# ARTIST-Association/ARTIST

Measured on AMD Instinct MI355X. Metric: traced rays/s fwd+bwd, 1000-heliostat NURBS field, higher is better.
Workload: dtype f32; 1 GPU; metric config: 1000 heliostats x 100 rays/point x 10000 points (1e+09 rays/step), 10x10 degree-3 NURBS, 256x256 bitmap, surface-reconstruction epoch fwd+bwd; heliostats=1000, rays_per_point=100, points_per_heliostat=10000, parallelism=heliostat-sharded dp1, heliostats_per_rank=1000

## Files before the change

artist_amd/csrc/flux_kernels.hip:

```cpp
#include <hip/hip_runtime.h>
#include <stdint.h>
#include <stdlib.h>
#include <mutex>
#include <vector>

#include "launch_common.hpp"
#include "flux_moments.hpp"

namespace art {

constexpr int kFluxBlock = 256;
constexpr int kReduceBlock = kMomentsBlock;

struct CropMap {
    float sx, sy, xc, yc;
    int W, Hh;
    __device__ __forceinline__ float ix(int j) const { return (((sx * lin11(j, W) + xc) + 1.0f) / 2.0f) * (float)(W - 1); }
    __device__ __forceinline__ float iy(int i) const { return (((sy * lin11(i, Hh) + yc) + 1.0f) / 2.0f) * (float)(Hh - 1); }
};

__device__ __forceinline__ CropMap make_map(const float* __restrict__ dims, float xc, float yc, int b, int W, int Hh, float crop_w,
                                            float crop_h)
{
    CropMap m;
// ... 112 lines not shown
#pragma unroll
        for (int q = 0; q < U; ++q) {
            if (k0 + q * (int)blockDim.x >= npx) break;
            float sx, sy;
            crop_sample_gradient(v[q], sx, sy);
            gx += (double)(go[q] * sx);
            gy += (double)(go[q] * sy);
        }
    }
    gx = block_sum(gx, s_red);
    gy = block_sum(gy, s_red);
    if (threadIdx.x == 0) finish_centre_gradient(gx, gy, W, Hh, gcom + 2 * b);
}

__device__ __forceinline__ float tap(float c, int p)
{
    const float c0 = floorf(c);
    const int p0 = (int)c0;
    const float t = c - c0;
    return p == p0 ? 1.0f - t : (p == p0 + 1 ? t : 0.0f);
}

template <int K>
__device__ __forceinline__ float gather_rows(const CropMap& m, const float* __restrict__ g, int W, int x, int y, int j0,
                                             int j1, int i0, int i1)
{
    float wx[K];
#pragma unroll
    for (int q = 0; q < K; ++q) wx[q] = j0 + q <= j1 ? tap(m.ix(j0 + q), x) : 0.0f;
    float acc = 0.0f;
    for (int i = i0; i <= i1; ++i) {
        const float wy = tap(m.iy(i), y);
        if (wy == 0.0f) continue;
        const float* __restrict__ grow = g + i * W + j0;
        float row = 0.0f;
#pragma unroll
        for (int q = 0; q < K; ++q)
            if (wx[q] != 0.0f) row += grow[q] * wx[q];
        acc += row * wy;
    }
    return acc;
}

__device__ __forceinline__ void tap_range(float scale, float centre, int n, int p, int& lo_i, int& hi_i)
{
    lo_i = 0; hi_i = n - 1;
    if (scale > 1e-6f && scale < 1e6f) {
        const float b = (centre + 1.0f) * 0.5f * (float)(n - 1) - scale * 0.5f * (float)(n - 1);
        const float lo = ((float)p - 1.004f - b) / scale, hi = ((float)p + 1.004f - b) / scale;
        if (lo > -2.0e9f && lo < 2.0e9f && hi > -2.0e9f && hi < 2.0e9f) { lo_i = max(0, (int)ceilf(lo)); hi_i = min(n - 1, (int)floorf(hi)); }
    }
}

__device__ __forceinline__ float crop_bwd_pixel(const CropMap& m, const float* __restrict__ g, float S,
                                                const float* __restrict__ gcom, int b, int Hh, int W, int x, int y)
{
    int j0, j1, i0, i1;
    tap_range(m.sx, m.xc, W, x, j0, j1);
    tap_range(m.sy, m.yc, Hh, y, i0, i1);
    float acc = 0.0f;
    if (j1 - j0 < 4) acc = gather_rows<4>(m, g, W, x, y, j0, j1, i0, i1);
    else if (j1 - j0 < 8) acc = gather_rows<8>(m, g, W, x, y, j0, j1, i0, i1);
    else {
        for (int i = i0; i <= i1; ++i) {
            const float wy = tap(m.iy(i), y);
            if (wy == 0.0f) continue;
            float row = 0.0f;
            for (int j = j0; j <= j1; ++j) {
                const float wx = tap(m.ix(j), x);
                if (wx != 0.0f) row += g[i * W + j] * wx;
            }
            acc += row * wy;
        }
    }
    return acc + gcom[2 * b] * (lin11(x, W) - m.xc) / S + gcom[2 * b + 1] * (lin11(y, Hh) - m.yc) / S;
}

constexpr int kTileX = 64, kTileY = 32, kTaps = 4, kTileRows = 64, kRowUnroll = 4;
template <bool LOSS>
__global__ __launch_bounds__(256) void flux_crop_bwd_tiled_kernel(const float* __restrict__ dims, const float* __restrict__ com,
                                                                  const float* __restrict__ gcom,
                                                                  const float* __restrict__ grad_out, int Hh, int W,
                                                                  float crop_w, float crop_h, float* __restrict__ grad_flux,
                                                                  const float* __restrict__ grad_loss, int grad_loss_stride)
{
    constexpr int CS = LOSS ? 4 : 3;
    __shared__ int s_j0[kTileX], s_i0[kTileY];
    __shared__ float s_wx[kTileX][kTaps], s_wy[kTileY][kTaps];
    __shared__ float s_t[kTileRows][kTileX];
    __shared__ int s_wide, s_ilo, s_ihi;
    __shared__ float s_gy[kTileY];
    const int b = blockIdx.z;
    const int x0 = blockIdx.x * kTileX, y0 = blockIdx.y * kTileY;
    const CropMap m = make_map(dims, com[CS * b], com[CS * b + 1], b, W, Hh, crop_w, crop_h);
    const float S = com[CS * b + 2];
    const float scale = LOSS ? (grad_loss[(int64_t)b * grad_loss_stride] * 2.0f) / com[CS * b + 3] : 1.0f;
    if (threadIdx.x == 0) { s_wide = 0; s_ilo = 0x7fffffff; s_ihi = -1; }
    __syncthreads();
    if (threadIdx.x < kTileX + kTileY) {
        const bool col = threadIdx.x < kTileX;
        const int t = col ? threadIdx.x : threadIdx.x - kTileX;
        const int p = col ? x0 + t : y0 + t;
        const int n = col ? W : Hh;
        int lo_i = 0, hi_i = -1;
        if (p < n) tap_range(col ? m.sx : m.sy, col ? m.xc : m.yc, n, p, lo_i, hi_i);
        if (hi_i - lo_i >= kTaps) s_wide = 1;
        (col ? s_j0 : s_i0)[t] = lo_i;
        for (int q = 0; q < kTaps; ++q) {
            const int o = lo_i + q;
            (col ? s_wx[t] : s_wy[t])[q] = o <= hi_i ? tap(col ? m.ix(o) : m.iy(o), p) : 0.0f;
        }
        if (!col && hi_i >= lo_i) { atomicMin(&s_ilo, lo_i); atomicMax(&s_ihi, hi_i); }
        if (!col) s_gy[t] = gcom[2 * b + 1] * (lin11(p, Hh) - m.yc) / S;
    }
    __syncthreads();
    const int ilo = s_ilo, ihi = s_ihi;
    const float* __restrict__ g = grad_out + (int64_t)b * Hh * W;
    if (s_wide || ihi - ilo >= kTileRows) {
        for (int k = threadIdx.x; k < kTileX * kTileY; k += 256) {
            const int x = x0 + (k & (kTileX - 1)), y = y0 + k / kTileX;
            if (x < W && y < Hh) grad_flux[((int64_t)b * Hh + y) * W + x] = scale * crop_bwd_pixel(m, g, S, gcom, b, Hh, W, x, y);
        }
        return;
    }
    const int tx = threadIdx.x & (kTileX - 1);
    const int x = x0 + tx;
    const bool in_x = x < W;
    const int j0 = s_j0[tx];
    const float wx0 = s_wx[tx][0], wx1 = s_wx[tx][1], wx2 = s_wx[tx][2], wx3 = s_wx[tx][3];
    const int c0 = min(j0, W - 1), c1 = min(j0 + 1, W - 1), c2 = min(j0 + 2, W - 1), c3 = min(j0 + 3, W - 1);
    const int xr = in_x ? 1 : 0;
    auto horizontal_pass = [&](auto&& row_sum) {
        for (int r = threadIdx.x / kTileX; r <= ihi - ilo; r += kRowUnroll * (256 / kTileX)) {
            float v[kRowUnroll];
#pragma unroll
            for (int q = 0; q < kRowUnroll; ++q) {
                const int rr = min(r + q * (256 / kTileX), ihi - ilo);
                v[q] = row_sum(g + (int64_t)(ilo + rr) * W);
            }
#pragma unroll
            for (int q = 0; q < kRowUnroll; ++q) {
                const int rr = r + q * (256 / kTileX);
                if (rr <= ihi - ilo) s_t[rr][tx] = in_x ? v[q] : 0.0f;
            }
        }
    };
    if (W >= 4) {
        struct __attribute__((packed, aligned(4))) Taps { float t0, t1, t2, t3; };
        const int cb = in_x ? min(j0, W - 4) : 0, sh = in_x ? j0 - cb : 0;
        const float w0 = sh == 0 ? wx0 : 0.0f, w1 = sh == 0 ? wx1 : (sh == 1 ? wx0 : 0.0f);
        const float w2 = sh == 0 ? wx2 : (sh == 1 ? wx1 : (sh == 2 ? wx0 : 0.0f));
        const float w3 = sh == 0 ? wx3 : (sh == 1 ? wx2 : (sh == 2 ? wx1 : wx0));
        horizontal_pass([&](const float* __restrict__ row) {
            const Taps t = *reinterpret_cast<const Taps*>(row + cb);
            return ((t.t0 * w0 + t.t1 * w1) + t.t2 * w2) + t.t3 * w3;
        });
    } else {
        horizontal_pass([&](const float* __restrict__ row) {
            return ((row[c0 * xr] * wx0 + row[c1 * xr] * wx1) + row[c2 * xr] * wx2) + row[c3 * xr] * wx3;
        });
    }
    __syncthreads();
    if (!in_x) return;
    const float gx = gcom[2 * b] * (lin11(x, W) - m.xc) / S;
    for (int ty = threadIdx.x / kTileX; ty < kTileY; ty += 256 / kTileX) {
        const int y = y0 + ty;
        if (y >= Hh) break;
        const int r0 = s_i0[ty] - ilo;
        float acc = 0.0f;
#pragma unroll
        for (int a = 0; a < kTaps; ++a) {
            const float wy = s_wy[ty][a];
            if (wy != 0.0f) acc += s_t[r0 + a][tx] * wy;
        }
        acc += gx + s_gy[ty];
        grad_flux[((int64_t)b * Hh + y) * W + x] = LOSS ? scale * acc : acc;
    }
}

template <typename F>
__device__ __forceinline__ void for_each_pair(const float* __restrict__ p, const float* __restrict__ g, int64_t npix, F&& f)
{
    const bool vec = (npix & 3) == 0 && ((reinterpret_cast<uintptr_t>(p) | reinterpret_cast<uintptr_t>(g)) & 15) == 0;
    if (vec) {
        const float4* __restrict__ p4 = reinterpret_cast<const float4*>(p);
        const float4* __restrict__ g4 = reinterpret_cast<const float4*>(g);
        for (int64_t k = threadIdx.x; k < (npix >> 2); k += blockDim.x) {
            const float4 a = p4[k], c = g4[k];
            f(4 * k, a.x, c.x); f(4 * k + 1, a.y, c.y); f(4 * k + 2, a.z, c.z); f(4 * k + 3, a.w, c.w);
        }
    } else {
        for (int64_t k = threadIdx.x; k < npix; k += blockDim.x) f(k, p[k], g[k]);
    }
}

struct KlNorms {
    static constexpr float eps = 1e-12f;
    float npf, ngf, dp, dg;
    __device__ __forceinline__ KlNorms(float np_, float ng_) : npf(np_), ngf(ng_), dp(fmaxf(np_, eps)), dg(fmaxf(ng_, eps)) {}
    __device__ __forceinline__ void term(float pk, float gk, double& acc, double& dot) const
    {
        const float t = logf(gk / dg + eps), q = logf(pk / dp + eps);
        const float et = expf(t);
        acc += (double)(et * (t - q));
        dot += (double)((-et / (pk / dp + eps)) * pk);
    }
    __device__ __forceinline__ float gradient(float pk, float gk, float dotf, float gl) const
    {
        const float t = logf(gk / dg + eps);
        const float a = -expf(t) / (pk / dp + eps);
        const float sgn = pk > 0.0f ? 1.0f : (pk < 0.0f ? -1.0f : 0.0f);
        const float through_norm = npf > eps ? sgn * dotf / (dp * dp) : 0.0f;
        return gl * (a / dp - through_norm);
    }
};

__global__ __launch_bounds__(kReduceBlock) void flux_loss_kernel(const float* __restrict__ pred, const float* __restrict__ truth,
                                                               int64_t npix, int mode, float* __restrict__ loss,
                                                               const float* __restrict__ grad_loss,
                                                               float* __restrict__ grad_pred)
{
    __shared__ double s_red[16];
    const int b = blockIdx.x;
    const float* __restrict__ p = pred + (int64_t)b * npix;
    const float* __restrict__ g = truth + (int64_t)b * npix;
    float* __restrict__ gp = grad_pred ? grad_pred + (int64_t)b * npix : nullptr;
    if (mode == 0) {
        double se = 0.0, sg = 0.0;
        for_each_pair(p, g, npix, [&](int64_t, float pk, float gk) { const float d = pk - gk; se += (double)(d * d); sg += (double)gk; });
        se = block_sum(se, s_red);
        const float sgf = (float)block_sum(sg, s_red);
        if (threadIdx.x == 0 && loss) loss[b] = (float)se / sgf;
        if (gp) {
            const float gl = grad_loss[b];
            for_each_pair(p, g, npix, [&](int64_t k, float pk, float gk) { gp[k] = gl * (2.0f * (pk - gk)) / sgf; });
        }
        return;
    }
    double np_ = 0.0, ng = 0.0;
    for_each_pair(p, g, npix, [&](int64_t, float pk, float gk) { np_ += (double)fabsf(pk); ng += (double)fabsf(gk); });
    const float npf = (float)block_sum(np_, s_red), ngf = (float)block_sum(ng, s_red);
    const KlNorms kl(npf, ngf);
    double acc = 0.0, dot = 0.0;
    for_each_pair(p, g, npix, [&](int64_t, float pk, float gk) { kl.term(pk, gk, acc, dot); });
    acc = block_sum(acc, s_red);
    const float dotf = (float)block_sum(dot, s_red);
    if (threadIdx.x == 0 && loss) loss[b] = (float)acc;
    if (gp) {
        const float gl = grad_loss[b];
        for_each_pair(p, g, npix, [&](int64_t k, float pk, float gk) { gp[k] = kl.gradient(pk, gk, dotf, gl); });
    }
}

constexpr int kMaxPartBitmaps = 512;
struct PartScratch { double com[kMaxPartBitmaps][kLossParts][3]; double acc[kMaxPartBitmaps][kLossParts][4]; };

__global__ __launch_bounds__(kReduceBlock) void flux_com_parts_kernel(const float* __restrict__ flux, int Hh, int W, int parts_per_wg,
                                                                    PartScratch* __restrict__ ws)
{
    __shared__ double s_red[16 * 4];
    const int b = blockIdx.y;
    const float* __restrict__ f = flux + (int64_t)b * Hh * W;
    for (int v = blockIdx.x * parts_per_wg; v < (int)(blockIdx.x + 1) * parts_per_wg; ++v) {
        double a[3];
        com_part_sums(f, Hh, W, v, s_red, a);
        if (threadIdx.x == 0) { ws->com[b][v][0] = a[0]; ws->com[b][v][1] = a[1]; ws->com[b][v][2] = a[2]; }
    }
}

__device__ __forceinline__ void com_from_parts(const double (*parts)[3], float& xc, float& yc, float& S)
{
    double s = 0.0, xs = 0.0, ys = 0.0;
    for (int v = 0; v < kLossParts; ++v) { s += parts[v][0]; xs += parts[v][1]; ys += parts[v][2]; }
    centre_from_sums(s, xs, ys, xc, yc, S);
}

__device__ __forceinline__ void loss_from_parts(const double (*acc)[4], float xc, float yc, float S, int b, int Hh, int W,
                                                float* __restrict__ loss, float* __restrict__ com4, float* __restrict__ gunit)
{
    double se = 0.0, sg = 0.0, gx = 0.0, gy = 0.0;
    for (int v = 0; v < kLossParts; ++v) { se += acc[v][0]; sg += acc[v][1]; gx += acc[v][2]; gy += acc[v][3]; }
    const float sgf = (float)sg;
    loss[b] = (float)se / sgf;
    com4[4 * b] = xc; com4[4 * b + 1] = yc; com4[4 * b + 2] = S; com4[4 * b + 3] = sgf;
    if (gunit) finish_centre_gradient(gx, gy, W, Hh, gunit + 2 * b);
}

template <bool WHOLE>
__global__ __launch_bounds__(kReduceBlock) void flux_crop_pixel_loss_fwd_kernel(const float* __restrict__ flux,
                                                                               const float* __restrict__ dims,
                                                                               const float* __restrict__ truth, int Hh, int W,
                                                                               float crop_w, float crop_h, int parts_per_wg,
                                                                               PartScratch* ws, float* __restrict__ residual,
                                                                               float* __restrict__ loss, float* __restrict__ com4,
                                                                               float* __restrict__ gunit, const double* __restrict__ moments,
                                                                               int stage_rows)
{
    extern __shared__ __attribute__((aligned(16))) float s_stage[];
    __shared__ double s_red[16 * 4];
    __shared__ double s_com[kLossParts][3], s_acc[kLossParts][4];
    const int b = blockIdx.y;
    const float* __restrict__ f = flux + (int64_t)b * Hh * W;
    const float* __restrict__ g = truth + (int64_t)b * Hh * W;
    float* __restrict__ res = residual ? residual + (int64_t)b * Hh * W : nullptr;
    float xc, yc, S;
    if (moments != nullptr) {
        com_from_parts(reinterpret_cast<const double(*)[3]>(moments + (int64_t)b * kLossParts * 3), xc, yc, S);
    } else if constexpr (WHOLE) {
        for (int v = 0; v < kLossParts; ++v) {
            double a[3];
            com_part_sums(f, Hh, W, v, s_red, a);
            if (threadIdx.x == 0) { s_com[v][0] = a[0]; s_com[v][1] = a[1]; s_com[v][2] = a[2]; }
        }
        __syncthreads();
        com_from_parts(s_com, xc, yc, S);
    } else {
        com_from_parts(ws->com[b], xc, yc, S);
    }
    const CropMap m = make_map(dims, xc, yc, b, W, Hh, crop_w, crop_h);
    for (int v = blockIdx.x * parts_per_wg; v < (int)(blockIdx.x + 1) * parts_per_wg; ++v) {
        int r0, r1;
        part_rows(Hh, v, r0, r1);
        double a[4] = {0.0, 0.0, 0.0, 0.0};
        if ((int)blockDim.x % W == 0) {
            const int j = threadIdx.x % W, di = blockDim.x / W;
            const CropAxis col = crop_column(m, j);
            int ylo = 0, nrows = 0;
            if (stage_rows > 0 && (W & 3) == 0) {
                const float ya_ = m.iy(r0), yb_ = m.iy(r1 - 1);
                if (ya_ > -1.0e9f && ya_ < 1.0e9f && yb_ > -1.0e9f && yb_ < 1.0e9f) {
                    ylo = max(0, (int)floorf(fminf(ya_, yb_)));
                    const int yhi = min(Hh - 1, (int)floorf(fmaxf(ya_, yb_)) + 1);
                    nrows = yhi - ylo + 1;
                    if (nrows > stage_rows) nrows = 0;
                }
            }
            constexpr int kRows = 4;
            auto rows = [&](auto&& pixel) {
            for (int i0 = r0 + threadIdx.x / W; i0 < r1; i0 += kRows * di) {
                float c[kRows], t[kRows], gxs[kRows], gys[kRows];
#pragma unroll
                for (int u = 0; u < kRows; ++u) {
                    const int i = min(i0 + u * di, r1 - 1);
                    CropTaps v;
                    c[u] = crop_sample_from(pixel, m, col, i, v);
                    t[u] = g[i * W + j];
                    crop_sample_gradient(v, gxs[u], gys[u]);
                }
#pragma unroll
                for (int u = 0; u < kRows; ++u) {
                    const int i = i0 + u * di;
                    if (i >= r1) break;
                    const float d = c[u] - t[u];
                    a[0] += (double)(d * d); a[1] += (double)t[u];
                    if (res) {
                        res[i * W + j] = d;
                        a[2] += (double)(d * gxs[u]);
                        a[3] += (double)(d * gys[u]);
                    }
                }
            }
            };
            if (nrows > 0) {
                __syncthreads();
                const float4* __restrict__ src = reinterpret_cast<const float4*>(f + (int64_t)ylo * W);
                float4* dst = reinterpret_cast<float4*>(s_stage);
                for (int k = threadIdx.x; k < nrows * (W >> 2); k += blockDim.x) dst[k] = src[k];
                __syncthreads();
                const float* staged = s_stage - ylo * W;
                rows([&](int k) { return staged[k]; });
            } else {
                rows([&](int k) { return f[k]; });
            }
        } else {
            for (int k = r0 * W + threadIdx.x; k < r1 * W; k += blockDim.x) {
                const int i = k / W, j = k - i * W;
                CropTaps v;
                const float c = crop_sample(f, m, crop_column(m, j), i, v);
                const float t = g[k];
                const float d = c - t;
                a[0] += (double)(d * d); a[1] += (double)t;
                if (res) {
                    float gxs, gys;
                    crop_sample_gradient(v, gxs, gys);
                    res[k] = d;
                    a[2] += (double)(d * gxs);
                    a[3] += (double)(d * gys);
                }
            }
        }
        block_sum_n<4>(a, s_red);
        if (threadIdx.x == 0) {
            double* out = WHOLE ? s_acc[v] : ws->acc[b][v];
            out[0] = a[0]; out[1] = a[1]; out[2] = a[2]; out[3] = a[3];
        }
    }
    if constexpr (WHOLE) {
        if (threadIdx.x == 0) loss_from_parts(s_acc, xc, yc, S, b, Hh, W, loss, com4, gunit);
    }
}

__global__ __launch_bounds__(256) void flux_crop_pixel_loss_final_kernel(const PartScratch* __restrict__ ws, int B, int Hh, int W,
                                                                         float* __restrict__ loss, float* __restrict__ com4,
                                                                         float* __restrict__ gunit, const double* __restrict__ moments)
{
    const int b = blockIdx.x * blockDim.x + threadIdx.x;
    if (b >= B) return;
    float xc, yc, S;
    com_from_parts(moments ? reinterpret_cast<const double(*)[3]>(moments + (int64_t)b * kLossParts * 3) : ws->com[b], xc, yc, S);
    loss_from_parts(ws->acc[b], xc, yc, S, b, Hh, W, loss, com4, gunit);
}

__global__ __launch_bounds__(kFluxBlock) void flux_com_px_bwd_kernel(const float* __restrict__ com, const float* __restrict__ grad_com,
                                                                     int Hh, int W, float* __restrict__ grad_flux)
{
    const int b = blockIdx.y;
    const int k = blockIdx.x * blockDim.x + threadIdx.x;
    if (k >= Hh * W) return;
    const int i = k / W, j = k - i * W;
    const float S = com[3 * b + 2];
    grad_flux[(int64_t)b * Hh * W + k] = (grad_com[2 * b] * ((float)j - com[3 * b]) + grad_com[2 * b + 1] * ((float)i - com[3 * b + 1])) / S;
}

template <typename F>
__device__ __forceinline__ void for_each_crop_pixel(const float* __restrict__ f, const CropMap& m, F&& fn)
{
    const int W = m.W, Hh = m.Hh;
    auto pixel = [&](int k, int i, const CropAxis& col) {
        CropTaps v;
        const float c = crop_sample(f, m, col, i, v);
        fn(k, c, v);
    };
    if ((int)blockDim.x % W == 0) {
        const int j = threadIdx.x % W, di = blockDim.x / W;
        const CropAxis col = crop_column(m, j);
#pragma unroll 4
        for (int i = threadIdx.x / W; i < Hh; i += di) pixel(i * W + j, i, col);
    } else {
        for (int k = threadIdx.x; k < Hh * W; k += blockDim.x) {
            const int i = k / W, j = k - i * W;
            pixel(k, i, crop_column(m, j));
        }
    }
}

__global__ __launch_bounds__(kReduceBlock) void flux_crop_kl_loss_fwd_kernel(const float* __restrict__ flux,
                                                                            const float* __restrict__ dims,
                                                                            const float* __restrict__ truth, int Hh, int W,
                                                                            float crop_w, float crop_h, float* __restrict__ loss,
                                                                            float* __restrict__ rec8)
{
    __shared__ double s_red[16 * 3];
    __shared__ float s_com[3];
    const int b = blockIdx.x;
    const float* __restrict__ f = flux + (int64_t)b * Hh * W;
    const float* __restrict__ g = truth + (int64_t)b * Hh * W;
    double sums[3];
// ... 11 lines not shown
    acc = block_sum(acc, s_red);
    const float dotf = (float)block_sum(dot, s_red);
    if (threadIdx.x == 0) {
        loss[b] = (float)acc;
        float* r = rec8 + 8 * b;
        r[0] = xc; r[1] = yc; r[2] = S; r[3] = npf; r[4] = ngf; r[5] = dotf; r[6] = 0.0f; r[7] = 0.0f;
    }
}

__global__ __launch_bounds__(kReduceBlock) void flux_crop_kl_loss_bwd_kernel(const float* __restrict__ flux,
                                                                            const float* __restrict__ dims,
                                                                            const float* __restrict__ truth,
                                                                            const float* __restrict__ rec8,
                                                                            const float* __restrict__ grad_loss, int Hh, int W,
                                                                            float crop_w, float crop_h,
                                                                            float* __restrict__ grad_crop, float* __restrict__ com3,
                                                                            float* __restrict__ gcom)
{
    __shared__ double s_red[16];
    const int b = blockIdx.x;
    const float* __restrict__ f = flux + (int64_t)b * Hh * W;
    const float* __restrict__ g = truth + (int64_t)b * Hh * W;
    float* __restrict__ gc = grad_crop + (int64_t)b * Hh * W;
    const float* r = rec8 + 8 * b;
    const CropMap m = make_map(dims, r[0], r[1], b, W, Hh, crop_w, crop_h);
    const KlNorms kl(r[3], r[4]);
    const float dotf = r[5], gl = grad_loss[b];
    double gx = 0.0, gy = 0.0;
    for_each_crop_pixel(f, m, [&](int k, float c, const CropTaps& v) {
        const float go = kl.gradient(c, g[k], dotf, gl);
        float sx, sy;
        crop_sample_gradient(v, sx, sy);
        gc[k] = go;
        gx += (double)(go * sx);
        gy += (double)(go * sy);
    });
    gx = block_sum(gx, s_red);
    gy = block_sum(gy, s_red);
    if (threadIdx.x == 0) {
        finish_centre_gradient(gx, gy, W, Hh, gcom + 2 * b);
        com3[3 * b] = m.xc; com3[3 * b + 1] = m.yc; com3[3 * b + 2] = r[2];
    }
}

}

using namespace art;

static PartScratch* flux_parts_scratch(hipStream_t stream)
{
    struct Entry { int dev; hipStream_t stream; PartScratch* ws; };
    static std::vector<Entry> table;
    static std::mutex lock;
    int dev = 0;
    if (hipGetDevice(&dev) != hipSuccess) return nullptr;
    std::lock_guard<std::mutex> guard(lock);
    for (const Entry& e : table)
        if (e.dev == dev && e.stream == stream) return e.ws;
    PartScratch* ws = nullptr;
    if (hipMalloc(reinterpret_cast<void**>(&ws), sizeof(PartScratch)) != hipSuccess) return nullptr;
    table.push_back({dev, stream, ws});
    return ws;
}

static int loss_workgroups_per_bitmap(int64_t B, int64_t Hh)
{
    const int forced = debug_env_int("ARTIST_HIP_LOSS_PARTS", 0);
    if (B > kMaxPartBitmaps || Hh < kLossParts) return 1;
    if (forced == 1 || forced == 2 || forced == 4) return forced;
    int cus = 256;
    {
        int dev = 0, n = 0;
        if (hipGetDevice(&dev) == hipSuccess && hipDeviceGetAttribute(&n, hipDeviceAttributeMultiprocessorCount, dev) == hipSuccess && n > 0)
            cus = n;
    }
    return 4 * B <= cus ? 4 : (2 * B <= cus ? 2 : 1);
}

template <bool LOSS>
static void launch_crop_bwd_tiled(hipStream_t stream, const float* dims, const float* com, const float* gcom, const float* grad_out,
                                  int64_t B, int64_t Hh, int64_t W, double crop_width, double crop_height, float* grad_flux,
                                  const float* grad_loss = nullptr, int64_t grad_loss_stride = 1)
{
    hipLaunchKernelGGL(flux_crop_bwd_tiled_kernel<LOSS>,
                       dim3((unsigned)((W + kTileX - 1) / kTileX), (unsigned)((Hh + kTileY - 1) / kTileY), (unsigned)B),
                       dim3(256), 0, stream, dims, com, gcom, grad_out, (int)Hh, (int)W, (float)crop_width, (float)crop_height,
                       grad_flux, grad_loss, (int)grad_loss_stride);
}

static bool crop_args_ok(const void* a, const void* b, const void* c, const void* d, int64_t B, int64_t Hh, int64_t W)
{
    return a && b && c && d && B >= 0 && Hh >= 1 && W >= 1 && Hh <= 65535 && Hh * W <= (int64_t)1 << 30 && B <= 65535;
}

static bool empty_batch(int64_t B, int64_t Hh, int64_t W)
{
    return B == 0 && Hh >= 1 && W >= 1;
}

extern "C" int art_flux_crop_fwd(const float* flux, const float* target_dims, int64_t B, int64_t Hh, int64_t W,
                                 double crop_width, double crop_height, float* out, float* centers, void* stream_)
{
    hipStream_t stream = static_cast<hipStream_t>(stream_);
    if (empty_batch(B, Hh, W)) return ART_OK;
    if (!crop_args_ok(flux, target_dims, out, centers, B, Hh, W)) return ART_EINVAL;
    hipLaunchKernelGGL(flux_com_kernel<NormalisedWeights>, dim3((unsigned)B), dim3(kReduceBlock), 0, stream, flux, (int)Hh, (int)W, centers);
    hipLaunchKernelGGL(flux_crop_fwd_kernel,
                       dim3((unsigned)((W + kFluxBlock - 1) / kFluxBlock), (unsigned)((Hh + kCropRows - 1) / kCropRows), (unsigned)B),
                       dim3(kFluxBlock), 0, stream, flux, target_dims, centers, (int)Hh, (int)W, (float)crop_width,
                       (float)crop_height, out);
    ART_HIP(hipGetLastError());
    return ART_OK;
}

extern "C" int art_flux_crop_bwd(const float* flux, const float* target_dims, const float* centers, int64_t B,
                                 int64_t Hh, int64_t W, double crop_width, double crop_height, const float* grad_out,
                                 float* grad_flux, float* workspace, void* stream_)
{
    hipStream_t stream = static_cast<hipStream_t>(stream_);
    if (empty_batch(B, Hh, W)) return ART_OK;
    if (!crop_args_ok(flux, target_dims, centers, grad_out, B, Hh, W) || !grad_flux || !workspace) return ART_EINVAL;
    hipLaunchKernelGGL(flux_crop_bwd_com_kernel, dim3((unsigned)B), dim3(kReduceBlock), 0, stream, flux, target_dims, centers,
                       grad_out, (int)Hh, (int)W, (float)crop_width, (float)crop_height, workspace);
    launch_crop_bwd_tiled<false>(stream, target_dims, centers, workspace, grad_out, B, Hh, W, crop_width, crop_height, grad_flux);
    ART_HIP(hipGetLastError());
    return ART_OK;
}

extern "C" int art_flux_loss(const float* prediction, const float* ground_truth, int64_t B, int64_t npix, int kind,
                             float* loss, const float* grad_loss, float* grad_prediction, void* stream_)
{
    hipStream_t stream = static_cast<hipStream_t>(stream_);
    if (empty_batch(B, npix, 1) && (kind == 0 || kind == 1)) return ART_OK;
    if (!prediction || !ground_truth || B < 0 || npix < 1 || (kind != 0 && kind != 1) || (!loss && !grad_prediction) ||
        (grad_prediction && !grad_loss))
        return ART_EINVAL;
    hipLaunchKernelGGL(flux_loss_kernel, dim3((unsigned)B), dim3(kReduceBlock), 0, stream, prediction, ground_truth, npix,
                       kind, loss, grad_loss, grad_prediction);
    ART_HIP(hipGetLastError());
    return ART_OK;
}

extern "C" int art_flux_crop_pixel_loss_fwd(const float* flux, const float* target_dims, const float* ground_truth, int64_t B,
                                            int64_t Hh, int64_t W, double crop_width, double crop_height, float* loss,
                                            float* centers4, float* residual, float* center_grad_unit, const double* moments,
                                            void* stream_)
{
    hipStream_t stream = static_cast<hipStream_t>(stream_);
    if (empty_batch(B, Hh, W)) return ART_OK;
    if (!crop_args_ok(flux, target_dims, ground_truth, loss, B, Hh, W) || !centers4 || (residual != nullptr) != (center_grad_unit != nullptr))
        return ART_EINVAL;
    const int P = loss_workgroups_per_bitmap(B, Hh);
    PartScratch* ws = P > 1 ? flux_parts_scratch(stream) : nullptr;
    int stage_rows = (int)std::min<int64_t>(Hh, (Hh + kLossParts - 1) / kLossParts + 4);
    if ((W & 3) != 0 || kReduceBlock % W != 0 || (int64_t)stage_rows * W * 4 > 76 * 1024) stage_rows = 0;
    const size_t stage_bytes = (size_t)stage_rows * W * sizeof(float);
    if (ws != nullptr) {
        if (moments == nullptr)
            hipLaunchKernelGGL(flux_com_parts_kernel, dim3((unsigned)P, (unsigned)B), dim3(kReduceBlock), 0, stream, flux, (int)Hh, (int)W,
                               kLossParts / P, ws);
        hipLaunchKernelGGL(flux_crop_pixel_loss_fwd_kernel<false>, dim3((unsigned)P, (unsigned)B), dim3(kReduceBlock), 0, stream, flux,
                           target_dims, ground_truth, (int)Hh, (int)W, (float)crop_width, (float)crop_height, kLossParts / P, ws, residual,
                           loss, centers4, center_grad_unit, moments, 0);
        hipLaunchKernelGGL(flux_crop_pixel_loss_final_kernel, dim3((unsigned)((B + 255) / 256)), dim3(256), 0, stream, ws, (int)B, (int)Hh,
                           (int)W, loss, centers4, center_grad_unit, moments);
    } else
    {
        if (stage_bytes > 48 * 1024)
            ART_HIP(hipFuncSetAttribute(reinterpret_cast<const void*>(&flux_crop_pixel_loss_fwd_kernel<true>),
                                        hipFuncAttributeMaxDynamicSharedMemorySize, (int)stage_bytes));
        hipLaunchKernelGGL(flux_crop_pixel_loss_fwd_kernel<true>, dim3(1u, (unsigned)B), dim3(kReduceBlock), stage_bytes, stream, flux, target_dims,
                           ground_truth, (int)Hh, (int)W, (float)crop_width, (float)crop_height, kLossParts, (PartScratch*)nullptr, residual,
                           loss, centers4, center_grad_unit, moments, stage_rows);
    }
    ART_HIP(hipGetLastError());
    return ART_OK;
}

extern "C" int art_flux_crop_pixel_loss_bwd(const float* target_dims, const float* centers4, const float* grad_loss,
                                            int64_t grad_loss_stride, const float* residual, const float* center_grad_unit, int64_t B,
                                            int64_t Hh, int64_t W, double crop_width, double crop_height, float* grad_flux, void* stream_)
{
    hipStream_t stream = static_cast<hipStream_t>(stream_);
    if (empty_batch(B, Hh, W)) return ART_OK;
    if (!crop_args_ok(residual, target_dims, center_grad_unit, centers4, B, Hh, W) || !grad_loss || !grad_flux ||
        (grad_loss_stride != 0 && grad_loss_stride != 1))
        return ART_EINVAL;
    launch_crop_bwd_tiled<true>(stream, target_dims, centers4, center_grad_unit, residual, B, Hh, W, crop_width, crop_height, grad_flux,
                                grad_loss, grad_loss_stride);
    ART_HIP(hipGetLastError());
    return ART_OK;
}

extern "C" int art_flux_center_of_mass(const float* flux, int64_t B, int64_t Hh, int64_t W, float* com, void* stream_)
{
    hipStream_t stream = static_cast<hipStream_t>(stream_);
    if (empty_batch(B, Hh, W)) return ART_OK;
    if (!crop_args_ok(flux, com, flux, com, B, Hh, W)) return ART_EINVAL;
    hipLaunchKernelGGL(flux_com_kernel<PixelWeights>, dim3((unsigned)B), dim3(kReduceBlock), 0, stream, flux, (int)Hh, (int)W, com);
    ART_HIP(hipGetLastError());
    return ART_OK;
}

extern "C" int art_flux_center_of_mass_bwd(const float* com, const float* grad_com, int64_t B, int64_t Hh, int64_t W,
                                           float* grad_flux, void* stream_)
{
    hipStream_t stream = static_cast<hipStream_t>(stream_);
    if (empty_batch(B, Hh, W)) return ART_OK;
    if (!crop_args_ok(com, grad_com, grad_flux, com, B, Hh, W)) return ART_EINVAL;
    hipLaunchKernelGGL(flux_com_px_bwd_kernel, dim3((unsigned)((Hh * W + kFluxBlock - 1) / kFluxBlock), (unsigned)B), dim3(kFluxBlock),
                       0, stream, com, grad_com, (int)Hh, (int)W, grad_flux);
    ART_HIP(hipGetLastError());
    return ART_OK;
}

extern "C" int art_flux_crop_kl_loss_fwd(const float* flux, const float* target_dims, const float* ground_truth, int64_t B,
                                         int64_t Hh, int64_t W, double crop_width, double crop_height, float* loss,
                                         float* record8, void* stream_)
{
    hipStream_t stream = static_cast<hipStream_t>(stream_);
    if (empty_batch(B, Hh, W)) return ART_OK;
    if (!crop_args_ok(flux, target_dims, ground_truth, loss, B, Hh, W) || !record8) return ART_EINVAL;
    hipLaunchKernelGGL(flux_crop_kl_loss_fwd_kernel, dim3((unsigned)B), dim3(kReduceBlock), 0, stream, flux, target_dims,
                       ground_truth, (int)Hh, (int)W, (float)crop_width, (float)crop_height, loss, record8);
    ART_HIP(hipGetLastError());
    return ART_OK;
}

extern "C" int art_flux_crop_kl_loss_bwd(const float* flux, const float* target_dims, const float* ground_truth,
                                         const float* record8, const float* grad_loss, int64_t B, int64_t Hh, int64_t W,
                                         double crop_width, double crop_height, float* grad_flux, float* workspace,
                                         void* stream_)
{
    hipStream_t stream = static_cast<hipStream_t>(stream_);
    if (empty_batch(B, Hh, W)) return ART_OK;
    if (!crop_args_ok(flux, target_dims, ground_truth, record8, B, Hh, W) || !grad_loss || !grad_flux || !workspace) return ART_EINVAL;
    float* grad_crop = workspace;
    float* com3 = workspace + B * Hh * W;
    float* gcom = com3 + 3 * B;
    hipLaunchKernelGGL(flux_crop_kl_loss_bwd_kernel, dim3((unsigned)B), dim3(kReduceBlock), 0, stream, flux, target_dims,
                       ground_truth, record8, grad_loss, (int)Hh, (int)W, (float)crop_width, (float)crop_height, grad_crop, com3,
                       gcom);
    launch_crop_bwd_tiled<false>(stream, target_dims, com3, gcom, grad_crop, B, Hh, W, crop_width, crop_height, grad_flux);
    ART_HIP(hipGetLastError());
    return ART_OK;
}
```

artist_amd/csrc/trace_kernels.hip:

```cpp
#include <hip/hip_runtime.h>
#include <algorithm>
#include <atomic>
#include <functional>
#include <cstdio>
#include <mutex>
#include <vector>
#include <stdint.h>
#include <stdlib.h>

#include <type_traits>

#define ART_TIMELINE_RECORDS_HERE
#include "trace_common.hpp"
#include "flux_moments.hpp"

namespace art {

__device__ __forceinline__ unsigned cvt_nearest_u32(float x)
{
    int q;
    asm("v_cvt_rpi_i32_f32_e32 %0, %1" : "=v"(q) : "v"(x));
    return (unsigned)q;
}

// ... 2362 lines not shown
                                                            int64_t npix, float sign_unit)
{
    const int64_t i = ((int64_t)blockIdx.x * blockDim.x + threadIdx.x) * 2;
    if (i + 1 < npix) {
        const ulonglong2 v = *reinterpret_cast<const ulonglong2*>(accum + i);
        *reinterpret_cast<float2*>(flux + i) = make_float2((float)v.x * sign_unit, (float)v.y * sign_unit);
        if ((v.x | v.y) != 0ull) *reinterpret_cast<ulonglong2*>(accum + i) = make_ulonglong2(0ull, 0ull);
    } else if (i < npix) {
        const unsigned long long v = accum[i];
        flux[i] = (float)v * sign_unit;
        if (v != 0ull) accum[i] = 0ull;
    }
}

__global__ __launch_bounds__(kMomentsBlock) void accum_to_flux_moments_kernel(unsigned long long* __restrict__ accum, float* __restrict__ flux,
                                                                             int Hh, int W, float sign_unit, double* __restrict__ moments)
{
    __shared__ double s_red[16 * 3];
    const int v = blockIdx.x;
    const int64_t map = blockIdx.y;
    unsigned long long* __restrict__ acc = accum + map * Hh * W;
    float* __restrict__ out = flux + map * Hh * W;
    auto load4 = [&](int64_t k) {
        const ulonglong2 lo = *reinterpret_cast<const ulonglong2*>(acc + 4 * k), hi = *reinterpret_cast<const ulonglong2*>(acc + 4 * k + 2);
        const float4 q = make_float4((float)lo.x * sign_unit, (float)lo.y * sign_unit, (float)hi.x * sign_unit, (float)hi.y * sign_unit);
        reinterpret_cast<float4*>(out)[k] = q;
        if ((lo.x | lo.y) != 0ull) *reinterpret_cast<ulonglong2*>(acc + 4 * k) = make_ulonglong2(0ull, 0ull);
        if ((hi.x | hi.y) != 0ull) *reinterpret_cast<ulonglong2*>(acc + 4 * k + 2) = make_ulonglong2(0ull, 0ull);
        return q;
    };
    auto load1 = [&](int64_t k) {
        const unsigned long long a1 = acc[k];
        const float q = (float)a1 * sign_unit;
        out[k] = q;
        if (a1 != 0ull) acc[k] = 0ull;
        return q;
    };
    double s, xs, ys;
    com_part_sums_from(load4, load1, Hh, W, v, s_red, s, xs, ys);
    if (threadIdx.x == 0) {
        double* m = moments + (map * kLossParts + v) * 3;
        m[0] = s; m[1] = xs; m[2] = ys;
    }
}

template <int VEC>
__global__ __launch_bounds__(256) void per_target_sum_kernel(const float* __restrict__ bitmaps,
                                                             const int32_t* __restrict__ target_idx, int H, int T,
                                                             int64_t npix, float* __restrict__ out)
{
    const int64_t i = ((int64_t)blockIdx.x * blockDim.x + threadIdx.x) * VEC;
    if (i >= npix) return;
    const int t = blockIdx.y;
    float acc[VEC];
#pragma unroll
    for (int v = 0; v < VEC; ++v) acc[v] = 0.0f;
    constexpr int kInFlight = VEC == 1 ? 64 : 8;
    for (int h0 = 0; h0 < H; h0 += kInFlight) {
        float val[kInFlight][VEC];
#pragma unroll
        for (int q = 0; q < kInFlight; ++q) {
            const int h = h0 + q;
            const bool mine = h < H && target_idx[h] == t;
#pragma unroll
            for (int v = 0; v < VEC; ++v) val[q][v] = 0.0f;
            if (mine) {
                if constexpr (VEC == 4) {
                    const float4 x = *reinterpret_cast<const float4*>(bitmaps + (int64_t)h * npix + i);
                    val[q][0] = x.x; val[q][1] = x.y; val[q][2] = x.z; val[q][3] = x.w;
                } else {
                    val[q][0] = bitmaps[(int64_t)h * npix + i];
                }
            }
        }
#pragma unroll
        for (int q = 0; q < kInFlight; ++q)
#pragma unroll
            for (int v = 0; v < VEC; ++v) acc[v] += val[q][v];
    }
#pragma unroll
    for (int v = 0; v < VEC; ++v) out[(int64_t)t * npix + i + v] = acc[v];
}

static void choose_chunks(TraceArgs& a, int target_blocks, int min_chunk)
{
    const int64_t base = (int64_t)a.H * a.n_ptiles;
    int64_t want = (target_blocks + base - 1) / (base > 0 ? base : 1);
    if (want < 1) want = 1;
    int chunk = (int)((a.R + want - 1) / want);
    if (chunk < min_chunk) chunk = min_chunk;
    if (chunk > a.R) chunk = a.R;
    a.r_chunk = chunk;
    a.n_rchunks = (a.R + chunk - 1) / chunk;
}

struct FwdConfig {
    int variant;
    int block;
    int tile_cap;
    int target_blocks;
    int min_chunk;
    int p_block;
    int p_block_bwd;
    bool p_block_fixed, p_block_bwd_fixed;
    int multipass_ratio;
    int min_rays;
    bool exact_pblock;
    int facet_points;
};

static FwdConfig fwd_config()
{
    FwdConfig c;
    const char* v = debug_env_str("ARTIST_HIP_FWD");
    c.variant = (v && v[0] == 'g') ? 1 : 0;
    c.block = debug_env_int("ARTIST_HIP_FWD_BLOCK", 1024);
    if (c.block < 64 || c.block > 1024 || (c.block % 64) != 0) c.block = 1024;
    int kb = debug_env_int("ARTIST_HIP_FWD_TILE_KB", 158);
    if (kb < 4) kb = 4;
    if (kb > 158) kb = 158;
    c.tile_cap = kb * 256;
    c.target_blocks = debug_env_int("ARTIST_HIP_FWD_BLOCKS", 512);
    c.min_chunk = debug_env_int("ARTIST_HIP_FWD_MINCHUNK", 4);
    c.min_rays = debug_env_int("ARTIST_HIP_FWD_MINRAYS", 100000);
    c.multipass_ratio = debug_env_int("ARTIST_HIP_FWD_MULTIPASS", 8);
    if (c.multipass_ratio < 1) c.multipass_ratio = 1;
    c.p_block_fixed = debug_env_str("ARTIST_HIP_FWD_PBLOCK") != nullptr;
    c.p_block_bwd_fixed = debug_env_str("ARTIST_HIP_BWD_PBLOCK") != nullptr;
    c.p_block = debug_env_int("ARTIST_HIP_FWD_PBLOCK", 1024);
    if (c.p_block < 64) c.p_block = 64;
    c.exact_pblock = debug_env_int("ARTIST_HIP_PBLOCK_EXACT", 1) != 0;
    c.facet_points = 0;
    c.p_block_bwd = debug_env_int("ARTIST_HIP_BWD_PBLOCK", 2048);
    if (c.p_block_bwd < 64) c.p_block_bwd = 64;
    return c;
}

static void window_geometry_for(TraceArgs& a, const FwdConfig& cfg, int p_block_target);

static unsigned* stream_work_counters(hipStream_t stream)
{
    struct Entry { int dev; hipStream_t stream; unsigned* base; };
    static std::vector<Entry> table;
    static unsigned* page = nullptr;
    static int page_dev = -1, page_used = 0;
    static std::mutex lock;
    constexpr int kPageEntries = 4096 / (int)(sizeof(unsigned) * kCountersPerStream);
    int dev = 0;
    if (hipGetDevice(&dev) != hipSuccess) return nullptr;
    std::lock_guard<std::mutex> guard(lock);
    for (const Entry& e : table)
        if (e.dev == dev && e.stream == stream) return e.base;
    if (page == nullptr || page_dev != dev || page_used == kPageEntries) {
        unsigned* fresh = nullptr;
        if (hipMalloc(reinterpret_cast<void**>(&fresh), 4096) != hipSuccess) return nullptr;
        if (hipMemset(fresh, 0, 4096) != hipSuccess) { (void)hipFree(fresh); return nullptr; }
        page = fresh; page_dev = dev; page_used = 0;
    }
    unsigned* base = page + (page_used++) * kCountersPerStream;
    table.push_back({dev, stream, base});
    return base;
}


struct SideStream {
    hipStream_t side = nullptr; hipEvent_t fork = nullptr, join = nullptr; int dev = -1; bool pending = false;
// ... 575 lines not shown
            const int threads = std::min(cfg.block, CY ? kCylBwdThreads : (BL ? (LN ? kLeanBlockBwdThreads : kBlockingBwdThreads) : 1024)); \
            const int rc = launch_bwd_lds<IL, AT, CY, BL, LN>(a, grad_flux, go, gn, prim_slabs, work_counter, blocks, threads, lds, stream); \
            if (rc != ART_OK) return rc;                                                                         \
        } while (0)
#define ART_LAUNCH_BWD_BL(CY, BL, LN)                                                                            \
        do {                                                                                                     \
            if (il && atomic_out) ART_LAUNCH_BWD(true, true, CY, BL, LN);                                        \
            else if (il) ART_LAUNCH_BWD(true, false, CY, BL, LN);                                                \
            else if (atomic_out) ART_LAUNCH_BWD(false, true, CY, BL, LN);                                        \
            else ART_LAUNCH_BWD(false, false, CY, BL, LN);                                                       \
        } while (0)
#define ART_LAUNCH_BWD_TYPE(CY)                                                                                  \
        do {                                                                                                     \
            if (blocking) ART_LAUNCH_BWD_BL(CY, true, false); else ART_LAUNCH_BWD_BL(CY, false, false);          \
        } while (0)
        if (T > 0 && Tc == 0 && lean) ART_LAUNCH_BWD_BL(false, false, true);
        else if (lean_block) ART_LAUNCH_BWD_BL(false, true, true);
        else
        if (T > 0 && !planar_done) ART_LAUNCH_BWD_TYPE(false);
        if (planar_done) a.split = 3;
        if (Tc > 0 && !blocking && debug_env_int("ARTIST_HIP_LEAN", 1) != 0 && debug_env_int("ARTIST_HIP_CYL_LEAN", 1) != 0) ART_LAUNCH_BWD_BL(true, false, true);
        else
        if (Tc > 0) ART_LAUNCH_BWD_TYPE(true);
#undef ART_LAUNCH_BWD_TYPE
#undef ART_LAUNCH_BWD_BL
#undef ART_LAUNCH_BWD
        ART_HIP(hipGetLastError());
        ART_HIP(diag::dump_timeline("ART_TIMELINE_OUT_BWD", items, stream));
        if (launch_lean) { const int rc = launch_lean(); if (rc != ART_OK) return rc; }
        if (blocking) {
            if (side.s) { side.s->end(); side.s = nullptr; }
            hipLaunchKernelGGL(reduce_prim_grads_kernel, dim3((unsigned)N), dim3(256), 0, stream, prim_slabs, a.wide_grad, a.cand, a.cand_count, a.H,
                               a.Cmax, a.n_pblocks * a.n_rchunks, grad_prim_corners, grad_prim_spans, grad_prim_normals);
            ART_HIP(hipGetLastError());
        }
        if (atomic_out) {
            const int64_t n = H * P;
            hipLaunchKernelGGL(reduce_chunks_kernel, dim3((unsigned)((n + 255) / 256)), dim3(256), 0, stream, go, gn, a.n_rchunks, n,
                               reinterpret_cast<float4*>(grad_origins), reinterpret_cast<float4*>(grad_normals));
            ART_HIP(hipGetLastError());
        }
        return ART_OK;
    }
    if (Tc > 0 || blocking) return ART_EUNSUPPORTED;
    a.r_chunk = a.R; a.n_rchunks = 1;
    const int64_t blocks = (int64_t)a.H * a.n_ptiles;
    if (blocks > 2147483647LL) return ART_EINVAL;
    if (il) hipLaunchKernelGGL(trace_bwd_kernel<true>, dim3((unsigned)blocks), dim3(kBlock), 0, stream, a, grad_flux, go, gn);
    else hipLaunchKernelGGL(trace_bwd_kernel<false>, dim3((unsigned)blocks), dim3(kBlock), 0, stream, a, grad_flux, go, gn);
    ART_HIP(hipGetLastError());
    return ART_OK;
}

extern "C" int64_t art_trace_bwd_scratch_need(int64_t H, int64_t R, int64_t P, int64_t facet_points, int64_t T, int64_t Tc, int64_t Cmax)
{
    if (H <= 0 || R <= 0 || P <= 0 || H > (1 << 24) || R > (1 << 24) || P > (1 << 26) || Cmax < 0 || Cmax > (1 << 22) || T < 0 || Tc < 0) return 0;
    FwdConfig cfg = fwd_config();
    if (cfg.variant != 0) return 0;
    if (facet_points < 0 || (facet_points > 0 && P % facet_points != 0)) return 0;
    const bool blocking = Cmax > 0;
    TraceArgs a = {};
    a.H = (int)H; a.R = (int)R; a.P = (int)P; a.Cmax = (int)Cmax;
    if (blocking && cfg.tile_cap > 148 * 256) cfg.tile_cap = 148 * 256;
    (void)bwd_main_geometry(a, cfg, bwd_uses_lean(blocking, T, Tc), bwd_uses_lean_block(blocking, T, Tc), facet_points, false);
    const BwdScratch n = bwd_scratch_need(a, blocking, Cmax);
    return n.chunk_floats + n.slab_floats + n.wide_floats;
}

extern "C" int64_t art_trace_bwd_scratch_floats(int64_t H, int64_t R, int64_t P, int64_t facet_points, int64_t Cmax)
{
    int64_t most = 0;
    for (int cfgno = 0; cfgno < 3; ++cfgno)
        most = std::max(most, art_trace_bwd_scratch_need(H, R, P, facet_points, cfgno == 1 ? 0 : 1, cfgno == 0 ? 0 : 1, Cmax));
    return most;
}

extern "C" int art_per_target_sum(const float* bitmaps, const int32_t* target_idx, int64_t H, int64_t T,
                                  int64_t npix, float* out, void* stream_)
{
    hipStream_t stream = static_cast<hipStream_t>(stream_);
    if (!out || T <= 0 || npix <= 0 || H < 0 || T > 65535 || (H > 0 && (!bitmaps || !target_idx))) return ART_EINVAL;
    const bool vec4 = npix >= (int64_t)1 << 20 && (npix % 4) == 0 && (reinterpret_cast<uintptr_t>(bitmaps) % 16) == 0 &&
                      (reinterpret_cast<uintptr_t>(out) % 16) == 0;
    if (vec4)
        hipLaunchKernelGGL(per_target_sum_kernel<4>, dim3((unsigned)((npix / 4 + 255) / 256), (unsigned)T), dim3(256), 0,
                           stream, bitmaps, target_idx, (int)H, (int)T, npix, out);
    else
        hipLaunchKernelGGL(per_target_sum_kernel<1>, dim3((unsigned)((npix + 255) / 256), (unsigned)T), dim3(256), 0, stream,
                           bitmaps, target_idx, (int)H, (int)T, npix, out);
    ART_HIP(hipGetLastError());
    return ART_OK;
}

extern "C" int art_async_status(void* stream_, int clear)
{
    hipStream_t stream = static_cast<hipStream_t>(stream_);
    const StatusWord status = status_word();
    if (status.host == nullptr) { g_last_hip_error = (int)hipErrorOutOfMemory; return ART_ELAUNCH; }
    ART_HIP(hipStreamSynchronize(stream));
    const unsigned word = *status.host;
    if (clear) *status.host = 0u;
    return (word & 1u) ? ART_ETARGET : ((word & 2u) ? ART_ECANDIDATES : ((word & 4u) ? ART_EQUEUE : ART_OK));
}
```

Baseline: 131.4 billion rays/s.

## Vectorize flux loss/backward stores and add strip-based per-target bitmap sum

Adds a float4-wide store path to the tiled flux crop backward kernel, and a wave-local LDS exchange in the pixel-loss forward kernel so ground-truth loads and residual stores are 16-byte coalesced. It also adds a new per-target sum kernel that has 1024-thread blocks cooperatively load many heliostat bitmaps for a 256-pixel strip, with software prefetch of the next round. The aim is to cut global memory transaction count and raise bandwidth use in these reduction and elementwise stages. The new paths raise LDS use, reduce the shared memory left for staging in the forward kernel, and are gated by alignment and env-var checks.

```diff
diff --git a/artist_amd/csrc/flux_kernels.hip b/artist_amd/csrc/flux_kernels.hip
--- a/artist_amd/csrc/flux_kernels.hip
+++ b/artist_amd/csrc/flux_kernels.hip
@@ -218,12 +218,13 @@
                                                                   const float* __restrict__ gcom,
                                                                   const float* __restrict__ grad_out, int Hh, int W,
                                                                   float crop_w, float crop_h, float* __restrict__ grad_flux,
-                                                                  const float* __restrict__ grad_loss, int grad_loss_stride)
+                                                                  const float* __restrict__ grad_loss, int grad_loss_stride,
+                                                                  int wide_store)
 {
     constexpr int CS = LOSS ? 4 : 3;
     __shared__ int s_j0[kTileX], s_i0[kTileY];
     __shared__ float s_wx[kTileX][kTaps], s_wy[kTileY][kTaps];
-    __shared__ float s_t[kTileRows][kTileX];
+    __shared__ __attribute__((aligned(16))) float s_t[kTileRows][kTileX];
     __shared__ int s_wide, s_ilo, s_ihi;
     __shared__ float s_gy[kTileY];
     const int b = blockIdx.z;
@@ -297,6 +298,36 @@
         });
     }
     __syncthreads();
+    if (wide_store) {
+        const int c4 = (threadIdx.x & 15) * 4;
+        if (x0 + c4 >= W) return;
+        float gx4[4];
+#pragma unroll
+        for (int k = 0; k < 4; ++k) gx4[k] = gcom[2 * b] * (lin11(x0 + c4 + k, W) - m.xc) / S;
+#pragma unroll
+        for (int ty = threadIdx.x >> 4; ty < kTileY; ty += 16) {
+            const int y = y0 + ty;
+            if (y >= Hh) break;
+            const int r0 = s_i0[ty] - ilo;
+            float acc[4] = {0.0f, 0.0f, 0.0f, 0.0f};
+#pragma unroll
+            for (int a = 0; a < kTaps; ++a) {
+                const float wy = s_wy[ty][a];
+                if (wy != 0.0f) {
+                    const float4 t = *reinterpret_cast<const float4*>(&s_t[r0 + a][c4]);
+                    acc[0] += t.x * wy; acc[1] += t.y * wy; acc[2] += t.z * wy; acc[3] += t.w * wy;
+                }
+            }
+            const float gy = s_gy[ty];
+#pragma unroll
+            for (int k = 0; k < 4; ++k) {
+                acc[k] += gx4[k] + gy;
+                if (LOSS) acc[k] = scale * acc[k];
+            }
+            *reinterpret_cast<float4*>(grad_flux + ((int64_t)b * Hh + y) * W + x0 + c4) = make_float4(acc[0], acc[1], acc[2], acc[3]);
+        }
+        return;
+    }
     if (!in_x) return;
     const float gx = gcom[2 * b] * (lin11(x, W) - m.xc) / S;
     for (int ty = threadIdx.x / kTileX; ty < kTileY; ty += 256 / kTileX) {
@@ -422,7 +453,7 @@
     if (gunit) finish_centre_gradient(gx, gy, W, Hh, gunit + 2 * b);
 }
 
-template <bool WHOLE>
+template <bool WHOLE, bool WIDE>
 __global__ __launch_bounds__(kReduceBlock) void flux_crop_pixel_loss_fwd_kernel(const float* __restrict__ flux,
                                                                                const float* __restrict__ dims,
                                                                                const float* __restrict__ truth, int Hh, int W,
@@ -432,6 +463,7 @@
                                                                                float* __restrict__ gunit, const double* __restrict__ moments,
                                                                                int stage_rows)
 {
+    constexpr int xchg_floats = WIDE ? kReduceBlock * 4 : 0;
     extern __shared__ __attribute__((aligned(16))) float s_stage[];
     __shared__ double s_red[16 * 4];
     __shared__ double s_com[kLossParts][3], s_acc[kLossParts][4];
@@ -458,7 +490,7 @@
         int r0, r1;
         part_rows(Hh, v, r0, r1);
         double a[4] = {0.0, 0.0, 0.0, 0.0};
-        if ((int)blockDim.x % W == 0) {
+        if (WIDE || (int)blockDim.x % W == 0) {
             const int j = threadIdx.x % W, di = blockDim.x / W;
             const CropAxis col = crop_column(m, j);
             int ylo = 0, nrows = 0;
@@ -497,18 +529,57 @@
                 }
             }
             };
+            auto rows_wide = [&](auto&& pixel) {
+                const int lane = threadIdx.x & 63, u4 = lane >> 4;
+                float* xb = s_stage + (threadIdx.x >> 6) * (kRows * 64);
+                const int c4 = (int)(threadIdx.x & ~63u) % W + 4 * (lane & 15);
+                auto segment = [&](int i0) { return min(i0 + u4 * di, r1 - 1) * W + c4; };
+                auto wave_sync = [] {
+                    __builtin_amdgcn_fence(__ATOMIC_RELEASE, "wavefront");
+                    __builtin_amdgcn_wave_barrier();
+                    __builtin_amdgcn_fence(__ATOMIC_ACQUIRE, "wavefront");
+                };
+                for (int i0 = r0 + threadIdx.x / W; i0 < r1; i0 += kRows * di) {
+                    *reinterpret_cast<float4*>(xb + 4 * lane) = *reinterpret_cast<const float4*>(g + segment(i0));
+                    wave_sync();
+                    float t[kRows];
+#pragma unroll
+                    for (int u = 0; u < kRows; ++u) t[u] = xb[u * 64 + lane];
+                    wave_sync();
+#pragma unroll
+                    for (int u = 0; u < kRows; ++u) {
+                        const int i = i0 + u * di;
+                        if (i >= r1) break;
+                        CropTaps v;
+                        float gxs, gys;
+                        const float c = crop_sample_from(pixel, m, col, i, v);
+                        crop_sample_gradient(v, gxs, gys);
+                        const float d = c - t[u];
+                        a[0] += (double)(d * d); a[1] += (double)t[u];
+                        xb[u * 64 + lane] = d;
+                        a[2] += (double)(d * gxs);
+                        a[3] += (double)(d * gys);
+                    }
+                    wave_sync();
+                    const float4 dv = *reinterpret_cast<const float4*>(xb + 4 * lane);
+                    if (i0 + u4 * di < r1) *reinterpret_cast<float4*>(res + (i0 + u4 * di) * W + c4) = dv;
+                    wave_sync();
+                }
+            };
             if (nrows > 0) {
                 __syncthreads();
                 const float4* __restrict__ src = reinterpret_cast<const float4*>(f + (int64_t)ylo * W);
-                float4* dst = reinterpret_cast<float4*>(s_stage);
+                float4* dst = reinterpret_cast<float4*>(s_stage + xchg_floats);
                 for (int k = threadIdx.x; k < nrows * (W >> 2); k += blockDim.x) dst[k] = src[k];
                 __syncthreads();
-                const float* staged = s_stage - ylo * W;
-                rows([&](int k) { return staged[k]; });
+                const float* staged = s_stage + xchg_floats - ylo * W;
+                if constexpr (WIDE) rows_wide([&](int k) { return staged[k]; });
+                else rows([&](int k) { return staged[k]; });
             } else {
-                rows([&](int k) { return f[k]; });
+                if constexpr (WIDE) rows_wide([&](int k) { return f[k]; });
+                else rows([&](int k) { return f[k]; });
             }
-        } else {
+        } else if constexpr (!WIDE) {
             for (int k = r0 * W + threadIdx.x; k < r1 * W; k += blockDim.x) {
                 const int i = k / W, j = k - i * W;
                 CropTaps v;
@@ -686,10 +757,11 @@
                                   int64_t B, int64_t Hh, int64_t W, double crop_width, double crop_height, float* grad_flux,
                                   const float* grad_loss = nullptr, int64_t grad_loss_stride = 1)
 {
+    const int wide_store = (W & 3) == 0 && (reinterpret_cast<uintptr_t>(grad_flux) & 15) == 0 && debug_env_int("ARTIST_HIP_FLUX_WIDE_BWD", 1) != 0;
     hipLaunchKernelGGL(flux_crop_bwd_tiled_kernel<LOSS>,
                        dim3((unsigned)((W + kTileX - 1) / kTileX), (unsigned)((Hh + kTileY - 1) / kTileY), (unsigned)B),
                        dim3(256), 0, stream, dims, com, gcom, grad_out, (int)Hh, (int)W, (float)crop_width, (float)crop_height,
-                       grad_flux, grad_loss, (int)grad_loss_stride);
+                       grad_flux, grad_loss, (int)grad_loss_stride, wide_store);
 }
 
 static bool crop_args_ok(const void* a, const void* b, const void* c, const void* d, int64_t B, int64_t Hh, int64_t W)
@@ -758,22 +830,27 @@
     PartScratch* ws = P > 1 ? flux_parts_scratch(stream) : nullptr;
     int stage_rows = (int)std::min<int64_t>(Hh, (Hh + kLossParts - 1) / kLossParts + 4);
     if ((W & 3) != 0 || kReduceBlock % W != 0 || (int64_t)stage_rows * W * 4 > 76 * 1024) stage_rows = 0;
-    const size_t stage_bytes = (size_t)stage_rows * W * sizeof(float);
+    const bool wide = ws == nullptr && residual != nullptr && W % 64 == 0 && kReduceBlock % W == 0 &&
+                      ((reinterpret_cast<uintptr_t>(ground_truth) | reinterpret_cast<uintptr_t>(residual)) & 15) == 0 &&
+                      debug_env_int("ARTIST_HIP_FLUX_WIDE_FWD", 1) != 0;
+    const int xchg_floats = wide ? kReduceBlock * 4 : 0;
+    if (wide && stage_rows > 0) stage_rows = (int)std::min<int64_t>(stage_rows, (76 * 1024 - xchg_floats * 4) / (W * 4));
+    const size_t stage_bytes = ((size_t)stage_rows * W + xchg_floats) * sizeof(float);
     if (ws != nullptr) {
         if (moments == nullptr)
             hipLaunchKernelGGL(flux_com_parts_kernel, dim3((unsigned)P, (unsigned)B), dim3(kReduceBlock), 0, stream, flux, (int)Hh, (int)W,
                                kLossParts / P, ws);
-        hipLaunchKernelGGL(flux_crop_pixel_loss_fwd_kernel<false>, dim3((unsigned)P, (unsigned)B), dim3(kReduceBlock), 0, stream, flux,
+        hipLaunchKernelGGL((flux_crop_pixel_loss_fwd_kernel<false, false>), dim3((unsigned)P, (unsigned)B), dim3(kReduceBlock), 0, stream, flux,
                            target_dims, ground_truth, (int)Hh, (int)W, (float)crop_width, (float)crop_height, kLossParts / P, ws, residual,
                            loss, centers4, center_grad_unit, moments, 0);
         hipLaunchKernelGGL(flux_crop_pixel_loss_final_kernel, dim3((unsigned)((B + 255) / 256)), dim3(256), 0, stream, ws, (int)B, (int)Hh,
                            (int)W, loss, centers4, center_grad_unit, moments);
     } else
     {
+        const auto kernel = wide ? &flux_crop_pixel_loss_fwd_kernel<true, true> : &flux_crop_pixel_loss_fwd_kernel<true, false>;
         if (stage_bytes > 48 * 1024)
-            ART_HIP(hipFuncSetAttribute(reinterpret_cast<const void*>(&flux_crop_pixel_loss_fwd_kernel<true>),
-                                        hipFuncAttributeMaxDynamicSharedMemorySize, (int)stage_bytes));
-        hipLaunchKernelGGL(flux_crop_pixel_loss_fwd_kernel<true>, dim3(1u, (unsigned)B), dim3(kReduceBlock), stage_bytes, stream, flux, target_dims,
+            ART_HIP(hipFuncSetAttribute(reinterpret_cast<const void*>(kernel), hipFuncAttributeMaxDynamicSharedMemorySize, (int)stage_bytes));
+        hipLaunchKernelGGL(kernel, dim3(1u, (unsigned)B), dim3(kReduceBlock), stage_bytes, stream, flux, target_dims,
                            ground_truth, (int)Hh, (int)W, (float)crop_width, (float)crop_height, kLossParts, (PartScratch*)nullptr, residual,
                            loss, centers4, center_grad_unit, moments, stage_rows);
     }
diff --git a/artist_amd/csrc/trace_kernels.hip b/artist_amd/csrc/trace_kernels.hip
--- a/artist_amd/csrc/trace_kernels.hip
+++ b/artist_amd/csrc/trace_kernels.hip
@@ -2468,6 +2468,42 @@
     for (int v = 0; v < VEC; ++v) out[(int64_t)t * npix + i + v] = acc[v];
 }
 
+template <int ROUND>
+__global__ __launch_bounds__(1024) void per_target_sum_strip_kernel(const float* __restrict__ bitmaps,
+                                                                    const int32_t* __restrict__ target_idx, int H, int T,
+                                                                    int64_t npix, float* __restrict__ out)
+{
+    constexpr int kPerWave = ROUND / 16;
+    __shared__ float4 s_slot[ROUND][64];
+    const int t = blockIdx.y, wave = threadIdx.x >> 6, lane = threadIdx.x & 63;
+    const int64_t strip = (int64_t)blockIdx.x * 256;
+    auto load_round = [&](int h0, float4 (&v)[kPerWave]) {
+#pragma unroll
+        for (int q = 0; q < kPerWave; ++q) {
+            const int h = h0 + wave + 16 * q;
+            v[q] = make_float4(0.0f, 0.0f, 0.0f, 0.0f);
+            if (h < H && target_idx[h] == t)
+                v[q] = reinterpret_cast<const float4*>(bitmaps + (int64_t)h * npix + strip)[lane];
+        }
+    };
+    float4 v[kPerWave];
+    load_round(0, v);
+    float acc = 0.0f;
+    for (int h0 = 0; h0 < H; h0 += ROUND) {
+#pragma unroll
+        for (int q = 0; q < kPerWave; ++q) s_slot[wave + 16 * q][lane] = v[q];
+        __syncthreads();
+        if (h0 + ROUND < H) load_round(h0 + ROUND, v);
+        if (threadIdx.x < 256) {
+            const float* __restrict__ s = reinterpret_cast<const float*>(s_slot) + threadIdx.x;
+#pragma unroll
+            for (int q = 0; q < ROUND; ++q) acc += s[q * 256];
+        }
+        __syncthreads();
+    }
+    if (threadIdx.x < 256) out[(int64_t)t * npix + strip + threadIdx.x] = acc;
+}
+
 static void choose_chunks(TraceArgs& a, int target_blocks, int min_chunk)
 {
     const int64_t base = (int64_t)a.H * a.n_ptiles;
@@ -3209,7 +3245,14 @@
     if (!out || T <= 0 || npix <= 0 || H < 0 || T > 65535 || (H > 0 && (!bitmaps || !target_idx))) return ART_EINVAL;
     const bool vec4 = npix >= (int64_t)1 << 20 && (npix % 4) == 0 && (reinterpret_cast<uintptr_t>(bitmaps) % 16) == 0 &&
                       (reinterpret_cast<uintptr_t>(out) % 16) == 0;
-    if (vec4)
+    const int strips = debug_env_int("ARTIST_HIP_PER_TARGET_WIDE", 1);
+    if (!vec4 && strips != 0 && H > 0 && (npix % 256) == 0 && (reinterpret_cast<uintptr_t>(bitmaps) % 16) == 0) {
+        const dim3 grid((unsigned)(npix / 256), (unsigned)T);
+        if (strips == 16)
+            hipLaunchKernelGGL(per_target_sum_strip_kernel<16>, grid, dim3(1024), 0, stream, bitmaps, target_idx, (int)H, (int)T, npix, out);
+        else
+            hipLaunchKernelGGL(per_target_sum_strip_kernel<32>, grid, dim3(1024), 0, stream, bitmaps, target_idx, (int)H, (int)T, npix, out);
+    } else if (vec4)
         hipLaunchKernelGGL(per_target_sum_kernel<4>, dim3((unsigned)((npix / 4 + 255) / 256), (unsigned)T), dim3(256), 0,
                            stream, bitmaps, target_idx, (int)H, (int)T, npix, out);
     else
```

After: 132.1 billion rays/s, median of 4. About the same (+0.5%).
